# yangsenwxy/VSR

Measured on AMD Instinct MI355X. Metric: voxels/sec fwd+bwd, 4× SR on 16×128×128 cine volumes, 1/2/4/8 MI355X, higher is better.
Workload: dtype bf16

## Files before the change

### vsr_amd/build.py

```python
from __future__ import annotations

import hashlib
import os
import re
import subprocess
from concurrent.futures import ThreadPoolExecutor
from pathlib import Path

ROOT = Path(__file__).resolve().parent
CSRC = ROOT / "csrc"
LIBDIR = ROOT / "_lib"
LIB = LIBDIR / "libvsrk.so"
INCLUDE = ROOT.parent / "include"
ARCH = os.environ.get("VSRK_ARCH", "gfx950")
HIPCC = os.environ.get("HIPCC", "/opt/rocm/bin/hipcc")
FLAGS = ["-O3", "-fPIC", "-std=c++17", f"--offload-arch={ARCH}", "-Wno-unused-result"]
SRC_FLAGS = {"conv_roll.hip": ["-fno-slp-vectorize"], "conv_roll_fold.hip": ["-fno-slp-vectorize"],
             "conv_wgrad_roll.hip": ["-fno-slp-vectorize"]}


def sources() -> list[Path]:
    return sorted(CSRC.glob("*.hip"))


def _digest() -> str:
    h = hashlib.sha256()
    for p in sources() + sorted(CSRC.glob("*.h")) + sorted(INCLUDE.glob("*.h")):
        h.update(p.name.encode())
        h.update(p.read_bytes())
    h.update(" ".join(FLAGS).encode())
    h.update(repr(sorted(SRC_FLAGS.items())).encode())
    return h.hexdigest()[:16]


_INC = re.compile(r'^\s*#\s*include\s+"([^"]+)"', re.M)


def _includes(src: Path) -> list[Path]:
    seen: dict[Path, None] = {}
    todo = [src]
    while todo:
        cur = todo.pop()
        for name in _INC.findall(cur.read_text()):
            p = (cur.parent / name).resolve()
            if p.exists() and p not in seen:
                seen[p] = None
                todo.append(p)
    return sorted(seen)


def is_current() -> bool:
    stamp = LIBDIR / "libvsrk.stamp"
    return LIB.exists() and stamp.exists() and stamp.read_text() == _digest()


def build(force: bool = False, verbose: bool = False) -> Path:
    LIBDIR.mkdir(exist_ok=True)
    stamp = LIBDIR / "libvsrk.stamp"
    digest = _digest()
    if not force and LIB.exists() and stamp.exists() and stamp.read_text() == digest:
        return LIB
    objdir = LIBDIR / "obj"
    objdir.mkdir(exist_ok=True)

    def compile_one(src: Path) -> Path:
        obj = objdir / (src.stem + ".o")
        deps = b"".join(p.read_bytes() for p in _includes(src))
        flags = FLAGS + SRC_FLAGS.get(src.name, [])
        key = hashlib.sha256(src.read_bytes() + deps + " ".join(flags).encode()).hexdigest()[:16]
        ostamp = objdir / (src.stem + ".stamp")
        if not force and obj.exists() and ostamp.exists() and ostamp.read_text() == key:
            return obj
        cmd = [HIPCC, *flags, "-I", str(INCLUDE), "-c", str(src), "-o", str(obj)]
        if verbose:
            print(" ".join(cmd), flush=True)
        r = subprocess.run(cmd, capture_output=True, text=True)
        if r.returncode != 0:
            raise RuntimeError(f"hipcc failed for {src.name}:\n{r.stderr[-6000:]}")
        ostamp.write_text(key)
        return obj

    with ThreadPoolExecutor(max_workers=min(8, len(sources()))) as ex:
        objs = list(ex.map(compile_one, sources()))
    tmp = LIB.with_suffix(".so.tmp")
    cmd = [HIPCC, "-shared", f"--offload-arch={ARCH}", *[str(o) for o in objs], "-o", str(tmp)]
    r = subprocess.run(cmd, capture_output=True, text=True)
    if r.returncode != 0:
        raise RuntimeError(f"link failed:\n{r.stderr[-6000:]}")
    os.replace(tmp, LIB)
    stamp.write_text(digest)
    return LIB


if __name__ == "__main__":
    print(build(force=True, verbose=True))
```

### vsr_amd/csrc/conv_fast.hip

```cpp
#include <cstdlib>
#include <string>
#include "conv_fast_impl.h"

namespace {
using namespace vsrk_conv;

int g_fast_mode = -1;

int num_cus_fast() {
  static int n = 0;
  if (n == 0) {
    int dev = 0;
    (void)hipGetDevice(&dev);
    if (hipDeviceGetAttribute(&n, hipDeviceAttributeMultiprocessorCount, dev) != hipSuccess || n <= 0) n = 256;
  }
  return n;
}

}

int vsrk_g_grid_cap = 0;

int vsrk_conv::fast_grid(int64_t ntiles) {
  int64_t g = std::min<int64_t>(ntiles, (int64_t)num_cus_fast());
  if (vsrk_g_grid_cap > 0) g = std::min<int64_t>(g, vsrk_g_grid_cap);
  return (int)std::max<int64_t>(g, 1);
}

extern "C" int vsrk_conv_set_algo(int32_t mode) {
  VSRK_CHECK(mode >= -1 && mode <= 1, "conv_set_algo: mode must be -1, 0 or 1");
  g_fast_mode = mode;
  return VSRK_OK;
}

extern int g_pw_wide_mode;

extern "C" int vsrk_conv_set_path(const char* path, int32_t mode) {
  VSRK_CHECK(path, "conv_set_path: null path");
  const std::string p(path);
  VSRK_CHECK(mode >= -1 && mode <= (p == "wgrad_row" || p == "roll_wr" ? 2 : 1),
             "conv_set_path: mode must be -1, 0 or 1 (wgrad_row, roll_wr: 2)");
  if (p == "fast") g_fast_mode = mode;
  else if (p == "thin") vsrk_g_thin_mode = mode;
  else if (p == "wgrad_pipe") vsrk_g_wgrad_pipe_mode = mode;
  else if (p == "pw") vsrk_g_pw_mode = mode;
  else if (p == "roll") vsrk_conv_set_roll_mode(mode);
  else if (p == "wgrad_roll") vsrk_conv_set_wgrad_roll_mode(mode);
  else if (p == "wgrad_row") vsrk_conv_set_wgrad_row_mode(mode);
  else if (p == "roll_wr") vsrk_conv_set_roll_wr_mode(mode);
  else if (p == "roll_fold") vsrk_conv_set_roll_fold_mode(mode);
  else if (p == "stencil") vsrk_conv_set_stencil_mode(mode);
  else if (p == "pw_wide") g_pw_wide_mode = mode;
  else VSRK_CHECK(false, "conv_set_path: unknown path '%s' (fast, pw, roll, roll_wr, roll_fold, thin, wgrad_pipe, wgrad_roll, wgrad_row, stencil)",
                  path);
  return VSRK_OK;
}

extern "C" int vsrk_conv_set_grid_cap(int32_t max_workgroups) {
  VSRK_CHECK(max_workgroups >= 0, "conv_set_grid_cap: max_workgroups must be >= 0");
  vsrk_g_grid_cap = max_workgroups;
  return VSRK_OK;
}

int vsrk_conv_fwd_fast(const vsrk_conv_desc* d, const vsrk_tensor5* x, const void* w_packed, const float* bias,
                       const float* pro_scale, const float* pro_shift, const vsrk_tensor5* residual,
                       const vsrk_tensor5* mask, const vsrk_tensor5* y, hipStream_t s) {
  if (g_fast_mode < 0) {
    const char* e = getenv("VSRK_CONV_FAST");
    g_fast_mode = (e && e[0] == '0') ? 0 : 1;
  }
  if (g_fast_mode == 0) return 0;
  if (!vsrk_is16(x->dtype)) return 0;
  if (const int rl = vsrk_conv_fwd_roll(d, x, w_packed, bias, pro_scale, pro_shift, residual, mask, y, s)) return rl;
  if (!chunk_ok(x, 2) || x->c % 8 != 0) return 0;
  const int xr = x->shuffle > 1 ? x->shuffle : 1, yr = y->shuffle > 1 ? y->shuffle : 1;
  if (xr > 1 && (x->c / (xr * xr)) % 32 != 0) return 0;
  if (yr > 1 && ((y->c / (yr * yr)) % 32 != 0 || residual || mask)) return 0;
  if (xr > 1 && d->prologue) return 0;
  if (d->kh != d->kw || (d->kh != 1 && d->kh != 3)) return 0;
  const int ye = vsrk_esize(y->dtype);
  if (((uintptr_t)y->ptr) % (4 * ye) != 0 || y->sn % 4 || y->sd % 4 || y->sh % 4 || y->sw % 4) return 0;
  if (y->c % 4 != 0 && !(y->c < 4 && !residual && !mask && !d->accumulate)) return 0;
  for (const vsrk_tensor5* t : {residual, mask}) {
    if (t && (((uintptr_t)t->ptr) % (4 * ye) != 0 || t->sn % 4 || t->sd % 4 || t->sh % 4 || t->sw % 4 ||
              t->shuffle > 1 || t->dtype != y->dtype))
      return 0;
  }
  FastArgs a;
  static int ablate = -1;
  if (ablate < 0) {
    const char* e = getenv("VSRK_FAST_ABLATE");
    ablate = e ? atoi(e) : 0;
  }
  a.ablate = ablate;
  a.x = make_view(x);
  a.y = make_view(y);
  a.res = residual ? make_view(residual) : a.y;
  a.msk = mask ? make_view(mask) : a.y;
  a.w = w_packed;
  a.bias = bias;
  a.pro_scale = pro_scale;
  a.pro_shift = pro_shift;
  a.cin = x->c;
  a.cout = y->c;
  a.cin_pad = round_up(x->c, 32);
  a.cout_pad = round_up(y->c, 128);
  a.kd = d->kd; a.pd = d->pd; a.ph = d->ph; a.pw = d->pw;
  a.prologue = d->prologue;
  a.act = d->act;
  a.accumulate = d->accumulate;
  a.has_res = residual != nullptr;
  a.has_mask = mask != nullptr;
  a.bias_r = d->bias_perm_r;
  a.out_scale = d->out_scale;
  a.act_param = d->act_param;
  a.mask_slope = d->mask_slope;
  a.tiles_w = ceil_div(y->w, TW);
  const int NT = y->c <= 32 ? 32 : (y->c <= 64 || d->kh == 3) ? 64 : 128;
  a.ntn = ceil_div(y->c, NT);
  const bool yf = y->dtype == VSRK_F32;
  const bool h16 = x->dtype == VSRK_F16;
  const bool ys = yr > 1, xs = xr > 1;
  int rc;
  if (d->kh == 1) {
    if (xs || ys) return 0;
    rc = fast_k1(a, NT, yf, h16, s);
  } else if (NT == 32) {
    if (xs || ys) return 0;
    rc = fast_k3_n32(a, yf, h16, s);
  } else if (!xs && !ys) {
    rc = fast_k3_n64(a, yf, h16, s);
  } else if (xs && !ys) {
    rc = fast_k3_n64_xs(a, yf, h16, s);
  } else if (!xs && ys) {
    rc = fast_k3_n64_ys(a, yf, h16, s);
  } else {
    return 0;
  }
  if (rc == kFastNotEligible) return 0;
  return rc == VSRK_OK ? 1 : -rc;
}
```

### vsr_amd/csrc/conv_roll.hip

```cpp
#include <cstdlib>
#include "conv_common.h"

#ifndef ROLL_NT
#define ROLL_NT 0
#endif
typedef uint32_t roll_u32x4 __attribute__((ext_vector_type(4)));
typedef int roll_v4i __attribute__((ext_vector_type(4)));
typedef __amdgpu_buffer_rsrc_t RRsrc;
constexpr uint32_t ROLL_OOB = 0x80000000u;
__device__ __forceinline__ RRsrc roll_rsrc(const void* base) {
  const uint64_t b = (uint64_t)base;
  const uint64_t u = ((uint64_t)(uint32_t)__builtin_amdgcn_readfirstlane((int)(uint32_t)(b >> 32)) << 32) |
                     (uint32_t)__builtin_amdgcn_readfirstlane((int)(uint32_t)b);
  return __builtin_amdgcn_make_buffer_rsrc((void*)u, 0, 0x7FFFFFF0, 0x00020000);
}
__device__ __forceinline__ uint4 roll_bload16(RRsrc r, uint32_t off) {
  return __builtin_bit_cast(uint4, __builtin_amdgcn_raw_buffer_load_b128(r, (int)off, 0, 0));
}
#ifndef ROLL_SWAP
#define ROLL_SWAP 1
#endif
#ifndef ROLL_PREF2D
#define ROLL_PREF2D 1
#endif
// ... 913 lines not shown
    return true;
  };
  while (step(std::integral_constant<int, 0>{}) && step(std::integral_constant<int, 1>{}) &&
         step(std::integral_constant<int, 2>{})) {
  }
  roll_wait_vmcnt<0>();
  if (ppre) settle();
  flush(ptl, pdi, true, ppre, fscr);
#ifdef ROLL_STAMP
  if (blockIdx.x < 16 && (wave == 0 || wave == 4)) {
    unsigned* o = g_roll_stamp + (blockIdx.x * 2 + (wave >> 2)) * 128;
    o[lane] = stv0;
    o[64 + lane] = stv1;
  }
#endif
  if constexpr (EM & RE_PMASK) slope_out(sacc);
}

__global__ __launch_bounds__(256) void roll_bnred_final_kernel(const float* __restrict__ ws, int ntiles, int ntn,
                                                               int cout, const float* __restrict__ invstd,
                                                               float* __restrict__ o1, float* __restrict__ o2) {
  const int c = blockIdx.x;
  if (c >= cout) return;
  const int blk = c >> 5, cc = c & 31;
  const int nt = (ntiles - blk + ntn - 1) / ntn;
  double s1 = 0.0, s2 = 0.0;
  constexpr int U = 8;
  const int n = nt * RNW;
  for (int i0 = threadIdx.x; i0 < n; i0 += 256 * U) {
    float v1[U], v2[U];
#pragma unroll
    for (int u = 0; u < U; ++u) {
      const int i = i0 + 256 * u;
      v1[u] = v2[u] = 0.f;
      if (i < n) {
        const int t = blk + ntn * (i / RNW), w = i % RNW;
        const float* p = ws + ((int64_t)t * RNW + w) * 64;
        v1[u] = p[cc];
        v2[u] = p[32 + cc];
      }
    }
#pragma unroll
    for (int u = 0; u < U; ++u) {
      s1 += v1[u];
      s2 += v2[u];
    }
  }
  __shared__ double r1[256], r2[256];
  r1[threadIdx.x] = s1;
  r2[threadIdx.x] = s2;
  __syncthreads();
  for (int k = 128; k > 0; k >>= 1) {
    if (threadIdx.x < k) {
      r1[threadIdx.x] += r1[threadIdx.x + k];
      r2[threadIdx.x] += r2[threadIdx.x + k];
    }
    __syncthreads();
  }
  if (threadIdx.x == 0) {
    o1[c] = (float)r1[0];
    o2[c] = (float)(r2[0] * (double)invstd[c]);
  }
}


int g_roll_mode = -1;
int g_roll_wr_mode = -1;

int roll_num_cus() {
  static int n = 0;
  if (n == 0) {
    int dev = 0;
    (void)hipGetDevice(&dev);
    if (hipDeviceGetAttribute(&n, hipDeviceAttributeMultiprocessorCount, dev) != hipSuccess || n <= 0) n = 256;
  }
  return n;
}

template <int KD, int NT, int PRO, int EM, int SP, typename H, int WR = 0>
int launch_roll(const RollArgs& a, size_t lds, int grid, hipStream_t s) {
  auto kern = conv_roll_kernel<KD, NT, PRO, EM, SP, H, WR>;
  (void)hipFuncSetAttribute((const void*)kern, hipFuncAttributeMaxDynamicSharedMemorySize, (int)lds);
  kern<<<grid, RNW * 64, lds, s>>>(a);
  VSRK_LAUNCH_CHECK("conv_fwd(roll)");
  return VSRK_OK;
}


}

#ifdef ROLL_FOLD_TU
int vsrk_conv_fwd_roll_fold(const vsrk_conv_desc* d, const vsrk_tensor5* x, const void* w_packed, const float* bias,
                            const float* pro_scale, const float* pro_shift, const vsrk_tensor5* y, hipStream_t s) {
  if (d->kd != 3 || d->kh != 3 || d->kw != 3 || d->pd != 0 || x->d != 3 || y->d != 1) return 0;
  if (!vsrk_is16(x->dtype) || y->dtype != x->dtype || x->shuffle > 1 || y->shuffle > 1) return 0;
  if (d->act != VSRK_ACT_NONE && d->act != VSRK_ACT_RELU) return 0;
  if (d->accumulate || d->mask_slope || d->bias_perm_r > 1) return 0;
  if (x->c % RCH != 0 || 3 * (x->c / RCH) > RMAXSUB || !chunk_ok(x, 2)) return 0;
  if (y->c % 32 != 0 || ((uintptr_t)y->ptr) % 16 != 0 || y->sn % 8 || y->sh % 8 || y->sw % 8) return 0;
  if (d->ph < 0 || d->ph > 2 || d->pw < 0 || d->pw > 2) return 0;
  if (y->h != x->h + 2 * d->ph - 2 || y->w != x->w + 2 * d->pw - 2 || y->n != x->n) return 0;
  for (const vsrk_tensor5* t : {x, y}) {
    const int64_t span = (int64_t)(t->n - 1) * t->sn + (int64_t)(t->d - 1) * t->sd +
                         (int64_t)(t->h + RFTH + 2) * t->sh + (int64_t)(t->w + 2 * RHW) * t->sw + t->c;
    if (span >= (1ll << 31) || t->sn < 0 || t->sd < 0 || t->sh < 0 || t->sw < 0) return 0;
  }
  RollArgs a;
  a.x.ptr = (char*)x->ptr;
  a.x.d = 1; a.x.h = x->h; a.x.w = x->w;
  a.x.sn = (int)x->sn; a.x.sd = (int)x->sd; a.x.sh = (int)x->sh; a.x.sw = (int)x->sw;
  a.y.ptr = (char*)y->ptr;
  a.y.d = 1; a.y.h = y->h; a.y.w = y->w;
  a.y.sn = (int)y->sn; a.y.sd = (int)y->sd; a.y.sh = (int)y->sh; a.y.sw = (int)y->sw;
  a.res = a.y;
  a.msk = a.y;
  a.w = w_packed;
  a.bias = bias;
  a.bias_r = 1;
  a.pro_scale = pro_scale;
  a.pro_shift = pro_shift;
  a.cin = 3 * x->c;
  a.cout = y->c;
  a.cin_pad = round_up(x->c, 32);
  a.cout_pad = round_up(y->c, 128);
  a.pd = 0;
  a.ph = d->ph;
  a.pw = d->pw;
  a.prologue = d->prologue;
  a.out_scale = d->out_scale;
  const int nc = x->c / RCH;
  a.nchunk = 3 * nc;
  a.fold_nc = nc;
  a.fold_wstride = 9 * a.cout_pad * a.cin_pad;
  a.fold_tab = 3 * x->c;
  a.fold_cin = x->c;
  a.act_param = nullptr;
  a.prio = 0;
  a.mask_slope = nullptr;
  a.slope_part = nullptr;
  for (int i = 0; i < a.nchunk; ++i) {
    const int kd = i / nc;
    a.spoff[i] = (int)(kd * x->sd + (i - kd * nc) * RCH);
    a.sptap[i] = (uint16_t)kd;
  }
  const int tiles_h = ceil_div(y->h, RFTH), tiles_w = ceil_div(y->w, TW), ntn = ceil_div(y->c, 32);
  const int64_t ntiles = (int64_t)y->n * tiles_h * tiles_w * ntn;
  if (ntiles == 0) return 1;
  VSRK_CHECK(ntiles < (1ll << 31), "conv_fwd(roll fold): too many tiles");
  a.dzc = 1;
  a.ntn = make_rdiv(ntn);
  a.nzc = make_rdiv(1);
  a.tiles_w = make_rdiv(tiles_w);
  a.tiles_h = make_rdiv(tiles_h);
  a.ntiles = (int)ntiles;
  using G = RollGeo<1, 1>;
  const size_t tables = (size_t)a.cout_pad * 4 + (d->prologue ? 2 * (size_t)a.fold_tab * 4 : 0);
  const size_t lds = (size_t)RNSLOT * G::SLOT + tables;
  if (lds > 160 * 1024) return 0;
  const int grid = (int)vsrk_capped_grid(std::min<int64_t>(ntiles, roll_num_cus()));
  const bool relu = d->act == VSRK_ACT_RELU;
  int rc = vsrk_dispatch16(x->dtype, [&](auto tag) {
    using H = decltype(tag);
    if (d->prologue)
      return relu ? launch_roll<1, 1, 1, RE_RELU, SP_FOLD, H>(a, lds, grid, s) : launch_roll<1, 1, 1, 0, SP_FOLD, H>(a, lds, grid, s);
    return relu ? launch_roll<1, 1, 0, RE_RELU, SP_FOLD, H>(a, lds, grid, s) : launch_roll<1, 1, 0, 0, SP_FOLD, H>(a, lds, grid, s);
  });
  if (rc == VSRK_ERR_UNSUPPORTED) return 0;
  return rc == VSRK_OK ? 1 : -rc;
}
#else

int vsrk_g_roll_dz = 0;

extern "C" int vsrk_conv_set_roll_depth(int32_t depths) {
  VSRK_CHECK(depths >= 0, "conv_set_roll_depth: depths must be >= 0");
  vsrk_g_roll_dz = depths;
  return VSRK_OK;
}

void vsrk_conv_set_roll_wr_mode(int mode) { g_roll_wr_mode = mode; }

void vsrk_conv_set_roll_mode(int mode) { g_roll_mode = mode; }

int g_roll_fold_mode = -1;
void vsrk_conv_set_roll_fold_mode(int mode) { g_roll_fold_mode = mode; }

size_t vsrk_roll_slope_ws_bytes() { return (size_t)roll_num_cus() * RNW * sizeof(double); }

static int roll_fwd_one(const vsrk_conv_desc* d, const vsrk_tensor5* x, const void* w_packed, const float* bias,
                        const float* pro_scale, const float* pro_shift, const vsrk_tensor5* residual,
                        const vsrk_tensor5* mask, const vsrk_tensor5* y, hipStream_t s, const vsrk_slope_out* slope,
                        vsrk_roll_bnred* bnred);

int vsrk_conv_fwd_roll(const vsrk_conv_desc* d, const vsrk_tensor5* x, const void* w_packed, const float* bias,
                       const float* pro_scale, const float* pro_shift, const vsrk_tensor5* residual,
                       const vsrk_tensor5* mask, const vsrk_tensor5* y, hipStream_t s, const vsrk_slope_out* slope,
                       vsrk_roll_bnred* bnred) {
  auto span = [](const vsrk_tensor5* t, int64_t n) -> int64_t {
    const int64_t r = t->shuffle > 1 ? t->shuffle : 1;
    return (n - 1) * t->sn + (int64_t)(t->d - 1) * t->sd + (int64_t)(r * (t->h + RFTH + 2) - 1) * t->sh +
           (int64_t)(r * (t->w + 2 * RHW) - 1) * t->sw + t->c;
  };
  const vsrk_tensor5* ts[4] = {x, y, residual, mask};
  auto fits = [&](int64_t n) {
    for (const vsrk_tensor5* t : ts)
      if (t && span(t, n) >= (1ll << 31)) return false;
    return true;
  };
  if (slope || bnred || x->n <= 1 || y->n != x->n || fits(x->n))
    return roll_fwd_one(d, x, w_packed, bias, pro_scale, pro_shift, residual, mask, y, s, slope, bnred);
  for (const vsrk_tensor5* t : ts)
    if (t && (t->n != x->n || t->sn < 0)) return 0;
  int nc = x->n;
  while (nc > 1 && !fits(nc)) nc = (nc + 1) / 2;
  if (!fits(nc)) return 0;
  for (int n0 = 0; n0 < x->n; n0 += nc) {
    vsrk_tensor5 c[4];
    for (int i = 0; i < 4; ++i) {
      if (!ts[i]) continue;
      c[i] = *ts[i];
      c[i].n = std::min(nc, x->n - n0);
      c[i].ptr = (char*)ts[i]->ptr + (int64_t)n0 * ts[i]->sn * vsrk_esize(ts[i]->dtype);
    }
    const int rc = roll_fwd_one(d, &c[0], w_packed, bias, pro_scale, pro_shift, residual ? &c[2] : nullptr,
                                mask ? &c[3] : nullptr, &c[1], s, nullptr, nullptr);
    if (rc == 0 && n0 == 0) return 0;
    if (rc == 0) return -VSRK_ERR_INVALID;
    if (rc < 0) return rc;
  }
  return 1;
}

static int roll_fwd_one(const vsrk_conv_desc* d, const vsrk_tensor5* x, const void* w_packed, const float* bias,
                        const float* pro_scale, const float* pro_shift, const vsrk_tensor5* residual,
                        const vsrk_tensor5* mask, const vsrk_tensor5* y, hipStream_t s, const vsrk_slope_out* slope,
                        vsrk_roll_bnred* bnred) {
  if (g_roll_mode < 0) {
    const char* e = getenv("VSRK_CONV_ROLL");
    g_roll_mode = !e ? 2 : (e[0] == '0' ? 0 : 1);
  }
  if (g_roll_fold_mode < 0) {
    const char* e = getenv("VSRK_ROLL_FOLD");
    g_roll_fold_mode = (e && e[0] == '0') ? 0 : 1;
  }
  if (g_roll_mode == 0) return 0;
  if (!vsrk_is16(x->dtype) || y->dtype != x->dtype) return 0;
  if (d->kh != 3 || d->kw != 3) return 0;
  const bool k3 = d->kd == 3;
  if (!k3 && !(d->kd == 1 && d->pd == 0 && y->c % 64 == 0)) return 0;
  const bool pmask = slope != nullptr;
  if ((d->bias_perm_r > 1 && (y->shuffle != d->bias_perm_r || y->c % (d->bias_perm_r * d->bias_perm_r))) ||
      (d->mask_slope && !pmask))
    return 0;
  if (pmask) {
    if (!mask || !d->mask_slope || residual || d->kd != 1 || d->prologue) return 0;
    if (mask->dtype != y->dtype || mask->shuffle != y->shuffle || mask->n != y->n || mask->d != y->d ||
        mask->h != y->h || mask->w != y->w || mask->c != y->c || mask->sn != y->sn ||
        (y->d > 1 && mask->sd != y->sd) ||
        mask->sh != y->sh || mask->sw != y->sw)
      return 0;
  }
  if (d->act == VSRK_ACT_PRELU && (k3 || !d->act_param)) return 0;
  if (k3 && (residual || mask || d->accumulate)) return 0;
  if (k3 && y->d == 1 && x->d == 3 && d->pd == 0 && !bnred && !residual && !mask && !pmask && g_roll_fold_mode != 0) {
    if (const int rf = vsrk_conv_fwd_roll_fold(d, x, w_packed, bias, pro_scale, pro_shift, y, s)) return rf;
  }
  if (g_roll_mode == 2 && k3 && y->d == 1 && !bnred && vsrk_g_roll_dz == 0) return 0;
  if (bnred) {
    const vsrk_tensor5* b = bnred->bnx;
    if (!k3 || d->prologue || d->act != VSRK_ACT_NONE || bias || d->out_scale != 1.f || !b || b->dtype != y->dtype ||
        b->shuffle > 1 ||
        b->n != y->n || b->d != y->d || b->h != y->h || b->w != y->w || b->c != y->c || b->sn != y->sn ||
        b->sd != y->sd || b->sh != y->sh || b->sw != y->sw)
      return 0;
  }
  const int sp = x->shuffle > 1 ? SP_X : (y->shuffle > 1 ? SP_Y : SP_NONE);
  if (x->shuffle > 1 && y->shuffle > 1) return 0;
  if (sp != SP_NONE) {
    if (k3 || d->prologue || residual || (mask && !pmask)) return 0;
    const vsrk_tensor5* t = sp == SP_X ? x : y;
    const int r = t->shuffle, cph = t->c / (r * r);
    if (cph * r * r != t->c || cph % (sp == SP_X ? RCH : 32) != 0) return 0;
    if (t->c / (sp == SP_X ? RCH : 32) > RMAXSUB) return 0;
  }
  if (x->c % RCH != 0 || !chunk_ok(x, 2)) return 0;
  if (d->pd < 0 || d->pd > 2 || d->ph < 0 || d->ph > 2 || d->pw < 0 || d->pw > 2) return 0;
  if (y->d != x->d + 2 * d->pd - (d->kd - 1) || y->h != x->h + 2 * d->ph - 2 || y->w != x->w + 2 * d->pw - 2) return 0;
  auto out_ok = [&](const vsrk_tensor5* t) {
    return t->dtype == y->dtype && (t->shuffle <= 1 || (t == y && sp == SP_Y)) && t->n == y->n && t->d == y->d &&
           t->h == y->h && t->w == y->w &&
           t->c == y->c && ((uintptr_t)t->ptr) % 8 == 0 && t->sn % 4 == 0 && t->sd % 4 == 0 && t->sh % 4 == 0 &&
           t->sw % 4 == 0;
  };
  if (y->c % (k3 ? 8 : 4) != 0 || !out_ok(y)) return 0;
  if ((residual && !out_ok(residual)) || (mask && !pmask && !out_ok(mask))) return 0;
  for (const vsrk_tensor5* t : {x, y, residual, mask}) {
    if (!t) continue;
    const int64_t r = t->shuffle > 1 ? t->shuffle : 1;
    const int64_t span = (int64_t)(t->n - 1) * t->sn + (int64_t)(t->d - 1) * t->sd +
                         (int64_t)(r * (t->h + RFTH + 2) - 1) * t->sh + (int64_t)(r * (t->w + 2 * RHW) - 1) * t->sw +
                         t->c;
    if (span >= (1ll << 31) || t->sn < 0 || t->sd < 0 || t->sh < 0 || t->sw < 0) return 0;
  }
  auto rview = [](const vsrk_tensor5* t) {
    RView v;
    const int r = t->shuffle > 1 ? t->shuffle : 1;
    v.ptr = (char*)t->ptr;
    v.d = t->d; v.h = t->h; v.w = t->w;
    v.sn = (int)t->sn; v.sd = (int)t->sd; v.sh = (int)(r * t->sh); v.sw = (int)(r * t->sw);
    return v;
  };
  RollArgs a;
  a.x = rview(x);
  a.y = rview(y);
  a.res = rview(residual ? residual : y);
  a.msk = rview(mask ? mask : y);
  a.w = w_packed;
  a.bias = bias;
  a.bias_r = d->bias_perm_r > 1 ? d->bias_perm_r : 1;
  a.pro_scale = pro_scale;
  a.pro_shift = pro_shift;
  a.cin = x->c;
  a.cout = y->c;
  a.cin_pad = round_up(x->c, 32);
  a.cout_pad = round_up(y->c, 128);
  a.pd = d->pd;
  a.ph = d->ph;
  a.pw = d->pw;
  a.prologue = d->prologue;
  a.out_scale = d->out_scale;
  a.nchunk = x->c / RCH;
  a.act_param = d->act_param;
  {
    static int prio = -1;
    if (prio < 0) {
      const char* e = getenv("VSRK_ROLL_PRIO");
      prio = (e && e[0] == '1') ? 1 : 0;
    }
    a.prio = prio;
  }
  if (sp != SP_NONE) {
    const vsrk_tensor5* t = sp == SP_X ? x : y;
    const int r = t->shuffle, cph = t->c / (r * r), step = sp == SP_X ? RCH : 32;
    for (int i = 0; i < t->c / step; ++i) {
      const int c = i * step, sub = c / cph, cc = c - sub * cph;
      a.spoff[i] = (int)((sub / r) * t->sh + (sub % r) * t->sw + cc);
      a.sptap[i] = subpixel_tapmask(d->subpixel, r, sub);
    }
  }
  const int nt = k3 ? 1 : 2;
  const int tiles_h = ceil_div(y->h, RFTH), tiles_w = ceil_div(y->w, TW), ntn = ceil_div(y->c, 32 * nt);
  const int64_t spatial = (int64_t)y->n * tiles_h * tiles_w * ntn;
  if (spatial == 0 || y->d == 0) return 1;
  int dzc = y->d;
  if (vsrk_g_roll_dz > 0) {
    dzc = std::min(vsrk_g_roll_dz, y->d);
  } else if (k3) {
    const int64_t want = 2 * (int64_t)roll_num_cus();
    if (spatial < want) {
      const int64_t runs = std::min<int64_t>(ceil_div64(want, spatial), y->d);
      dzc = (int)ceil_div64(y->d, runs);
    }
  } else {
    dzc = 1;
  }
  a.dzc = dzc;
  const int nzc = ceil_div(y->d, dzc);
  a.ntn = make_rdiv(ntn);
  a.nzc = make_rdiv(nzc);
  a.tiles_w = make_rdiv(tiles_w);
  a.tiles_h = make_rdiv(tiles_h);
  const int64_t ntiles = spatial * nzc;
  VSRK_CHECK(ntiles < (1ll << 31), "conv_fwd(roll): too many tiles");
  a.ntiles = (int)ntiles;
  if (g_roll_wr_mode < 0) {
    const char* e = getenv("VSRK_ROLL_WRES");
    g_roll_wr_mode = (e && e[0] == '0') ? 0 : 1;
  }
  const int wres_mode = g_roll_wr_mode;
  const size_t nb = k3 ? RollGeo<3, 1>::NB : RollGeo<1, 2>::NB;
  const size_t wbytes = (size_t)a.nchunk * nb * 1024;
  const size_t tables = (size_t)a.cout_pad * 4 + (d->prologue || bnred ? 2 * (size_t)a.cin_pad * 4 : 0) +
                        (bnred ? 4 * (size_t)a.cout_pad * 4 : 0);
  const size_t wslot = k3 ? RollGeo<3, 1, 1>::SLOT : RollGeo<1, 2, 1>::SLOT;
  const bool pref2d =
      wres_mode != 2 && !k3 && ((residual != nullptr) != (mask != nullptr && !pmask)) && !d->accumulate;
  const bool wr = wres_mode && sp == SP_NONE && !d->prologue && wbytes <= 80 * 1024 && !pref2d &&
                  (k3 ? dzc == y->d : ntn == 1) && (size_t)RNSLOT * wslot + wbytes + tables <= 160 * 1024;
  const size_t slot = wr ? wslot : (k3 ? RollGeo<3, 1>::SLOT : RollGeo<1, 2>::SLOT);
  const size_t lds = (size_t)RNSLOT * slot + (wr ? wbytes : 0) + tables;
  if (bnred) {
    if (bnred->ws_floats < (size_t)ntiles * RNW * 64) return 0;
    a.bnx = (const char*)bnred->bnx->ptr;
    a.msk = rview(bnred->bnx);
    a.bn_sc = bnred->scale;
    a.bn_sh = bnred->shift;
    a.bn_mu = bnred->mean;
    a.bn_is = bnred->invstd;
    a.red_ws = bnred->ws;
    bnred->ntiles = (int)ntiles;
    bnred->ntn = ntn;
  }
  if (lds > 160 * 1024) return 0;
  const int grid = (int)vsrk_capped_grid(std::min<int64_t>(ntiles, roll_num_cus()));
  const bool relu = d->act == VSRK_ACT_RELU;
  const int em = (residual ? RE_RES : 0) | (mask ? (pmask ? RE_PMASK : RE_MASK) : 0) | (d->accumulate ? RE_ACC : 0) |
                 (relu ? RE_RELU : 0) | (d->act == VSRK_ACT_PRELU ? RE_PRELU : 0);
  a.mask_slope = d->mask_slope;
  if (pmask) {
    if ((size_t)grid * RNW > slope->cap) return 0;
    a.slope_part = slope->part;
    *slope->nparts = grid * RNW;
  }
  int rc = vsrk_dispatch16(x->dtype, [&](auto tag) {
    using H = decltype(tag);
    if (k3) {
      if (bnred)
        return wr ? launch_roll<3, 1, 0, RE_BNRED, SP_NONE, H, 1>(a, lds, grid, s)
                  : launch_roll<3, 1, 0, RE_BNRED, SP_NONE, H>(a, lds, grid, s);
      if (d->prologue) return relu ? launch_roll<3, 1, 1, RE_RELU, SP_NONE, H>(a, lds, grid, s) : launch_roll<3, 1, 1, 0, SP_NONE, H>(a, lds, grid, s);
      if (wr)
        return relu ? launch_roll<3, 1, 0, RE_RELU, SP_NONE, H, 1>(a, lds, grid, s)
                    : launch_roll<3, 1, 0, 0, SP_NONE, H, 1>(a, lds, grid, s);
      return relu ? launch_roll<3, 1, 0, RE_RELU, SP_NONE, H>(a, lds, grid, s) : launch_roll<3, 1, 0, 0, SP_NONE, H>(a, lds, grid, s);
    }
    if (d->prologue) {
      if (sp != SP_NONE || em != 0) return (int)VSRK_ERR_UNSUPPORTED;
      return launch_roll<1, 2, 1, 0, SP_NONE, H>(a, lds, grid, s);
    }
    if (sp == SP_X) {
      switch (em) {
        case 0: return launch_roll<1, 2, 0, 0, SP_X, H>(a, lds, grid, s);
        case RE_PRELU: return launch_roll<1, 2, 0, RE_PRELU, SP_X, H>(a, lds, grid, s);
        case RE_ACC: return launch_roll<1, 2, 0, RE_ACC, SP_X, H>(a, lds, grid, s);
        case RE_PMASK: return launch_roll<1, 2, 0, RE_PMASK, SP_X, H>(a, lds, grid, s);
        case RE_PMASK | RE_ACC: return launch_roll<1, 2, 0, RE_PMASK | RE_ACC, SP_X, H>(a, lds, grid, s);
        default: return (int)VSRK_ERR_UNSUPPORTED;
      }
    }
    if (sp == SP_Y) {
      switch (em) {
        case 0: return launch_roll<1, 2, 0, 0, SP_Y, H>(a, lds, grid, s);
        case RE_PRELU: return launch_roll<1, 2, 0, RE_PRELU, SP_Y, H>(a, lds, grid, s);
        case RE_ACC: return launch_roll<1, 2, 0, RE_ACC, SP_Y, H>(a, lds, grid, s);
        case RE_PMASK: return launch_roll<1, 2, 0, RE_PMASK, SP_Y, H>(a, lds, grid, s);
        case RE_PMASK | RE_ACC: return launch_roll<1, 2, 0, RE_PMASK | RE_ACC, SP_Y, H>(a, lds, grid, s);
        default: return (int)VSRK_ERR_UNSUPPORTED;
      }
    }
    if (wr) {
      switch (em) {
        case 0: return launch_roll<1, 2, 0, 0, SP_NONE, H, 1>(a, lds, grid, s);
        case RE_RELU: return launch_roll<1, 2, 0, RE_RELU, SP_NONE, H, 1>(a, lds, grid, s);
        case RE_RES | RE_ACC: return launch_roll<1, 2, 0, RE_RES | RE_ACC, SP_NONE, H, 1>(a, lds, grid, s);
        case RE_PMASK: return launch_roll<1, 2, 0, RE_PMASK, SP_NONE, H, 1>(a, lds, grid, s);
        default: return (int)VSRK_ERR_UNSUPPORTED;
      }
    }
    switch (em) {
      case 0: return launch_roll<1, 2, 0, 0, SP_NONE, H>(a, lds, grid, s);
      case RE_RELU: return launch_roll<1, 2, 0, RE_RELU, SP_NONE, H>(a, lds, grid, s);
      case RE_RES: return launch_roll<1, 2, 0, RE_RES, SP_NONE, H>(a, lds, grid, s);
      case RE_MASK: return launch_roll<1, 2, 0, RE_MASK, SP_NONE, H>(a, lds, grid, s);
      case RE_RES | RE_ACC: return launch_roll<1, 2, 0, RE_RES | RE_ACC, SP_NONE, H>(a, lds, grid, s);
      case RE_PMASK: return launch_roll<1, 2, 0, RE_PMASK, SP_NONE, H>(a, lds, grid, s);
      default: return (int)VSRK_ERR_UNSUPPORTED;
    }
  });
  if (rc == VSRK_ERR_UNSUPPORTED) return 0;
  return rc == VSRK_OK ? 1 : -rc;
}

#ifdef ROLL_STAMP
extern "C" int vsrk_roll_stamps(unsigned* dst) {
  return hipMemcpyFromSymbol(dst, HIP_SYMBOL(g_roll_stamp), sizeof(g_roll_stamp)) == hipSuccess ? 0 : 1;
}
#endif

extern "C" size_t vsrk_conv_prelu_bwd_workspace(void) {
  return std::max(vsrk_roll_slope_ws_bytes(), vsrk_pw_pbwd_ws_bytes());
}

extern "C" int vsrk_conv_fwd_prelu_bwd(const vsrk_conv_desc* d, const vsrk_tensor5* x, const void* w_packed,
                                       const float* bias, const vsrk_tensor5* y_fwd, const vsrk_tensor5* y,
                                       int32_t c_lo, float* da, int32_t accumulate_da, void* workspace,
                                       size_t workspace_bytes, void* stream) {
  VSRK_CHECK(d && x && y && y_fwd && w_packed && d->mask_slope, "conv_fwd_prelu_bwd: null argument");
  VSRK_CHECK(workspace && workspace_bytes >= vsrk_conv_prelu_bwd_workspace(),
             "conv_fwd_prelu_bwd: workspace %zu < %zu bytes", workspace_bytes, vsrk_conv_prelu_bwd_workspace());
  VSRK_CHECK(((uintptr_t)workspace & 15) == 0, "conv_fwd_prelu_bwd: workspace must be 16-byte aligned");
  VSRK_CHECK(c_lo >= 0 && c_lo < y->c, "conv_fwd_prelu_bwd: c_lo %d outside [0, %d)", c_lo, y->c);
  hipStream_t s = (hipStream_t)stream;
  if ((int64_t)y->n * y->d * y->h * y->w == 0) {
    if (da && !accumulate_da) (void)hipMemsetAsync(da, 0, sizeof(float), s);
    return VSRK_OK;
  }
  int nparts = 0;
  const vsrk_slope_out so{(double*)workspace, workspace_bytes / sizeof(double), &nparts};
  int rc;
  if (d->kd == 1 && d->kh == 1 && d->kw == 1) {
    if (bias) return VSRK_ERR_UNSUPPORTED;
    rc = vsrk_conv_fwd_pw_pbwd(d, x, w_packed, y_fwd, y, c_lo, &so, s);
  } else {
    if (c_lo != 0) return VSRK_ERR_UNSUPPORTED;
    rc = vsrk_conv_fwd_roll(d, x, w_packed, bias, nullptr, nullptr, nullptr, y_fwd, y, s, &so);
  }
  if (rc == 0) return VSRK_ERR_UNSUPPORTED;
  if (rc < 0) return -rc;
  if (da) {
    vsrk_slope_final((const double*)workspace, nparts, d->mask_slope, da, accumulate_da, 0, s);
    VSRK_LAUNCH_CHECK("conv_fwd_prelu_bwd_final");
  }
  return VSRK_OK;
}

int vsrk_roll_bnred_final(const vsrk_roll_bnred& r, int cout, float* sum_dy, float* sum_dy_xhat, hipStream_t s) {
  roll_bnred_final_kernel<<<cout, 256, 0, s>>>(r.ws, r.ntiles, r.ntn, cout, r.invstd, sum_dy, sum_dy_xhat);
  VSRK_LAUNCH_CHECK("conv_fwd_reduce(roll) final");
  return VSRK_OK;
}

size_t vsrk_roll_bnred_ws_floats(const vsrk_tensor5* y) {
  return (size_t)y->n * ceil_div(y->h, RFTH) * ceil_div(y->w, TW) * ceil_div(y->c, 32) * std::max(y->d, 1) * RNW * 64;
}
#endif
```

### vsr_amd/csrc/vsrk_internal.h

```cpp
#pragma once
#include <algorithm>
#include "vsrk_common.h"

size_t vsrk_channel_reduce_ws_bytes(int c);
int vsrk_channel_reduce_internal(const vsrk_tensor5* x, int mode, int perm_r, float scale, float* sum,
                                 float* sumsq, int accumulate, void* ws, size_t ws_bytes, hipStream_t s);

int vsrk_conv_fwd_fast(const vsrk_conv_desc* d, const vsrk_tensor5* x, const void* w_packed, const float* bias,
                       const float* pro_scale, const float* pro_shift, const vsrk_tensor5* residual,
                       const vsrk_tensor5* mask, const vsrk_tensor5* y, hipStream_t s);
int vsrk_conv_fwd_stencil(const vsrk_conv_desc* d, const vsrk_tensor5* x, const void* w_packed, const float* bias,
                          const vsrk_tensor5* residual, const vsrk_tensor5* mask, const vsrk_tensor5* y,
                          hipStream_t s);
int vsrk_conv_fwd_stencil_out(const vsrk_conv_desc* d, const vsrk_tensor5* x, const void* w_packed,
                              const float* bias, const vsrk_tensor5* residual, const vsrk_tensor5* mask,
                              const vsrk_tensor5* y, hipStream_t s);
void vsrk_conv_set_stencil_mode(int mode);
int vsrk_conv_fwd_thin(const vsrk_conv_desc* d, const vsrk_tensor5* x, const void* w_packed, const float* bias,
                       const float* pro_scale, const float* pro_shift, const vsrk_tensor5* residual,
                       const vsrk_tensor5* mask, const vsrk_tensor5* y, hipStream_t s);

struct vsrk_roll_bnred {
  const vsrk_tensor5* bnx;
  const float *scale, *shift, *mean, *invstd;
  float* ws;
  size_t ws_floats;
  int ntiles, ntn;
};
struct vsrk_slope_out {
  double* part;
  size_t cap;
  int* nparts;
};
void vsrk_slope_final(const double* part, int nparts, const float* a, float* da, int accumulate, int pre,
                      hipStream_t s);
int vsrk_conv_fwd_roll(const vsrk_conv_desc* d, const vsrk_tensor5* x, const void* w_packed, const float* bias,
                       const float* pro_scale, const float* pro_shift, const vsrk_tensor5* residual,
                       const vsrk_tensor5* mask, const vsrk_tensor5* y, hipStream_t s,
                       const vsrk_slope_out* slope = nullptr, vsrk_roll_bnred* bnred = nullptr);
int vsrk_roll_bnred_final(const vsrk_roll_bnred& r, int cout, float* sum_dy, float* sum_dy_xhat, hipStream_t s);
size_t vsrk_roll_bnred_ws_floats(const vsrk_tensor5* y);
size_t vsrk_roll_slope_ws_bytes();
void vsrk_conv_set_roll_mode(int mode);
void vsrk_conv_set_roll_wr_mode(int mode);
void vsrk_conv_set_roll_fold_mode(int mode);
int vsrk_conv_fwd_roll_fold(const vsrk_conv_desc* d, const vsrk_tensor5* x, const void* w_packed, const float* bias,
                            const float* pro_scale, const float* pro_shift, const vsrk_tensor5* y, hipStream_t s);

int vsrk_conv_fwd_pw(const vsrk_conv_desc* d, const vsrk_tensor5* x, const void* w_packed, const float* bias,
                     const float* pro_scale, const float* pro_shift, const vsrk_tensor5* residual,
                     const vsrk_tensor5* mask, const vsrk_tensor5* y, hipStream_t s);
int vsrk_conv_fwd_pw_wide(const vsrk_conv_desc* d, const vsrk_tensor5* x, const void* w_packed, const float* bias,
                          const vsrk_tensor5* residual, const vsrk_tensor5* mask, const vsrk_tensor5* y,
                          hipStream_t s);
int vsrk_conv_fwd_pw_pbwd(const vsrk_conv_desc* d, const vsrk_tensor5* x, const void* w_packed,
                          const vsrk_tensor5* mask, const vsrk_tensor5* y, int c_lo, const vsrk_slope_out* slope,
                          hipStream_t s);
size_t vsrk_pw_pbwd_ws_bytes();
size_t vsrk_conv_wgrad_pw_workspace(const vsrk_conv_desc* d, const vsrk_tensor5* x, const vsrk_tensor5* dy);
int vsrk_conv_wgrad_pw(const vsrk_conv_desc* d, const vsrk_tensor5* x, const vsrk_tensor5* dy,
                       const float* pro_scale, const float* pro_shift, float dy_scale, int32_t perm_r, float* dw,
                       float* dbias, int32_t accumulate, void* workspace, size_t workspace_bytes, hipStream_t s);

extern int vsrk_g_pw_mode;
extern int vsrk_g_thin_mode;
extern int vsrk_g_wgrad_pipe_mode;
extern int vsrk_g_grid_cap;
static inline int64_t vsrk_capped_grid(int64_t g) {
  return vsrk_g_grid_cap > 0 ? std::max<int64_t>(1, std::min<int64_t>(g, vsrk_g_grid_cap)) : g;
}
```

Measured before the change: 57.75 million.

## Add row-streaming 3x3 conv kernel for 64-channel 2D convs in roll path

```diff
diff --git a/vsr_amd/build.py b/vsr_amd/build.py
--- a/vsr_amd/build.py
+++ b/vsr_amd/build.py
@@ -16,7 +16,7 @@
 HIPCC = os.environ.get("HIPCC", "/opt/rocm/bin/hipcc")
 FLAGS = ["-O3", "-fPIC", "-std=c++17", f"--offload-arch={ARCH}", "-Wno-unused-result"]
 SRC_FLAGS = {"conv_roll.hip": ["-fno-slp-vectorize"], "conv_roll_fold.hip": ["-fno-slp-vectorize"],
-             "conv_wgrad_roll.hip": ["-fno-slp-vectorize"]}
+             "conv_wgrad_roll.hip": ["-fno-slp-vectorize"], "conv_row.hip": ["-fno-slp-vectorize"]}
 
 
 def sources() -> list[Path]:
diff --git a/vsr_amd/csrc/conv_fast.hip b/vsr_amd/csrc/conv_fast.hip
--- a/vsr_amd/csrc/conv_fast.hip
+++ b/vsr_amd/csrc/conv_fast.hip
@@ -51,7 +51,8 @@
   else if (p == "roll_fold") vsrk_conv_set_roll_fold_mode(mode);
   else if (p == "stencil") vsrk_conv_set_stencil_mode(mode);
   else if (p == "pw_wide") g_pw_wide_mode = mode;
-  else VSRK_CHECK(false, "conv_set_path: unknown path '%s' (fast, pw, roll, roll_wr, roll_fold, thin, wgrad_pipe, wgrad_roll, wgrad_row, stencil)",
+  else if (p == "row") vsrk_conv_set_row_mode(mode);
+  else VSRK_CHECK(false, "conv_set_path: unknown path '%s' (fast, pw, pw_wide, roll, roll_wr, roll_fold, row, thin, wgrad_pipe, wgrad_roll, wgrad_row, stencil)",
                   path);
   return VSRK_OK;
 }
diff --git a/vsr_amd/csrc/conv_roll.hip b/vsr_amd/csrc/conv_roll.hip
--- a/vsr_amd/csrc/conv_roll.hip
+++ b/vsr_amd/csrc/conv_roll.hip
@@ -1239,6 +1239,13 @@
                          t->c;
     if (span >= (1ll << 31) || t->sn < 0 || t->sd < 0 || t->sh < 0 || t->sw < 0) return 0;
   }
+  if (g_roll_wr_mode < 0) {
+    const char* e = getenv("VSRK_ROLL_WRES");
+    g_roll_wr_mode = (e && e[0] == '0') ? 0 : 1;
+  }
+  if (!k3 && sp == SP_NONE && !pmask && !bnred && g_roll_wr_mode == 1) {
+    if (const int rw = vsrk_conv_fwd_row(d, x, w_packed, bias, residual, mask, y, s)) return rw;
+  }
   auto rview = [](const vsrk_tensor5* t) {
     RView v;
     const int r = t->shuffle > 1 ? t->shuffle : 1;
@@ -1310,10 +1317,6 @@
   const int64_t ntiles = spatial * nzc;
   VSRK_CHECK(ntiles < (1ll << 31), "conv_fwd(roll): too many tiles");
   a.ntiles = (int)ntiles;
-  if (g_roll_wr_mode < 0) {
-    const char* e = getenv("VSRK_ROLL_WRES");
-    g_roll_wr_mode = (e && e[0] == '0') ? 0 : 1;
-  }
   const int wres_mode = g_roll_wr_mode;
   const size_t nb = k3 ? RollGeo<3, 1>::NB : RollGeo<1, 2>::NB;
   const size_t wbytes = (size_t)a.nchunk * nb * 1024;
diff --git a/vsr_amd/csrc/conv_row.hip b/vsr_amd/csrc/conv_row.hip
--- /dev/null
+++ b/vsr_amd/csrc/conv_row.hip
@@ -0,0 +1,353 @@
+#include <cstdlib>
+#include "conv_common.h"
+
+namespace {
+using namespace vsrk_conv;
+
+constexpr int CR_NW = 8;
+constexpr int CR_SEG = 128;
+constexpr int CR_SLOT = (CR_SEG + 2) * 128;
+constexpr int CR_NSLOT = 4;
+constexpr int CR_BIAS = CR_NSLOT * CR_SLOT;
+constexpr int CR_LDS = CR_BIAS + 256;
+constexpr int CR_MINBAND = 4;
+constexpr uint32_t CR_OOB = 0x80000000u;
+enum { CE_RES = 1, CE_MASK = 2, CE_ACC = 4, CE_RELU = 8 };
+
+typedef __amdgpu_buffer_rsrc_t CrRsrc;
+typedef int cr_v4i __attribute__((ext_vector_type(4)));
+__device__ __forceinline__ CrRsrc cr_rsrc(const void* base) {
+  const uint64_t b = (uint64_t)base;
+  const uint64_t u = ((uint64_t)(uint32_t)__builtin_amdgcn_readfirstlane((int)(uint32_t)(b >> 32)) << 32) |
+                     (uint32_t)__builtin_amdgcn_readfirstlane((int)(uint32_t)b);
+  return __builtin_amdgcn_make_buffer_rsrc((void*)u, 0, 0x7FFFFFF0, 0x00020000);
+}
+__device__ __forceinline__ uint4 cr_load16(CrRsrc r, uint32_t voff, uint32_t soff) {
+  return __builtin_bit_cast(uint4, __builtin_amdgcn_raw_buffer_load_b128(r, (int)voff, (int)soff, 0));
+}
+__device__ __forceinline__ void cr_store16(CrRsrc r, uint32_t voff, uint4 v) {
+  __builtin_amdgcn_raw_buffer_store_b128(__builtin_bit_cast(cr_v4i, v), r, (int)voff, 0, 0);
+}
+
+struct CrView {
+  const char* ptr;
+  int64_t sn, sd;
+  int sh, sw;
+};
+
+struct ConvRowArgs {
+  CrView x, y, res, msk;
+  const void* w;
+  const float* bias;
+  int cout_pad, cin_pad;
+  float out_scale;
+  int D, H, W;
+  int nseg, nband, band_h, nitems;
+};
+
+template <int EM, bool HALO, typename H>
+__global__ __launch_bounds__(CR_NW * 64, 1) void conv_row_kernel(ConvRowArgs a) {
+  extern __shared__ __attribute__((aligned(16))) char lds[];
+  const int tid = threadIdx.x, lane = tid & 63, r = lane & 31, hf = lane >> 5;
+  const int wave = __builtin_amdgcn_readfirstlane(tid >> 6);
+  const int coh = wave & 1, vq = wave >> 1;
+
+  uint4 wf[9][4];
+  {
+    const H* wp = reinterpret_cast<const H*>(a.w);
+#pragma unroll
+    for (int t = 0; t < 9; ++t)
+#pragma unroll
+      for (int c = 0; c < 4; ++c)
+        wf[t][c] = *reinterpret_cast<const uint4*>(wp + ((int64_t)(t * a.cout_pad + coh * 32 + r) * a.cin_pad + c * 16 + 8 * hf));
+  }
+  const int ecc = 2 * (r >> 4) + hf;
+  const int ech = coh * 32 + 8 * ecc;
+  const float osc = a.out_scale;
+  float* lbias = reinterpret_cast<float*>(lds + CR_BIAS);
+  if (tid < 64) lbias[tid] = a.bias ? a.bias[tid] * osc : 0.f;
+  if constexpr (!HALO) {
+    if (tid < CR_NSLOT * 16)
+      *reinterpret_cast<uint4*>(lds + (tid >> 4) * CR_SLOT + ((tid >> 3) & 1) * (CR_SEG + 1) * 128 + (tid & 7) * 16) =
+          make_uint4(0, 0, 0, 0);
+  }
+
+  uint32_t fa[3], fh[3];
+#pragma unroll
+  for (int kw = 0; kw < 3; ++kw) {
+    const int lv = vq * 32 + r + kw, sz = (lv >> 1) & 7;
+    fa[kw] = (uint32_t)(lv * 128 + ((hf ^ (sz & 1)) << 4));
+    fh[kw] = (uint32_t)(sz >> 1);
+  }
+  const int sp = lane & 7;
+  constexpr int NSQ = HALO ? 3 : 2;
+  const int scol = 8 * wave + (lane >> 3);
+  const int hcol = (lane >> 3) == 0 ? -1 : CR_SEG;
+  const uint32_t sdst = (uint32_t)((scol + 1) * 128 + ((sp ^ (((scol + 1) >> 1) & 7)) << 4));
+  const uint32_t hdst = (uint32_t)((hcol + 1) * 128 + ((sp ^ (((hcol + 1) >> 1) & 7)) << 4));
+  const bool halo_lane = wave == 0 && lane < 16;
+
+  f32x16 b0, b1;
+
+  for (int item = blockIdx.x; item < a.nitems; item += gridDim.x) {
+    const int band = item % a.nband;
+    const int t1 = item / a.nband;
+    const int seg = t1 % a.nseg, img = t1 / a.nseg;
+    const int in_ = img / a.D, id = img - in_ * a.D;
+    const int c0 = seg * CR_SEG;
+    const int r0 = band * a.band_h, r1 = min(r0 + a.band_h, a.H);
+    const int nstage = r1 - r0 + 1;
+
+    const CrRsrc rx = cr_rsrc(reinterpret_cast<const H*>(a.x.ptr) + (in_ * a.x.sn + id * a.x.sd));
+    const CrRsrc ry = cr_rsrc(reinterpret_cast<const H*>(a.y.ptr) + (in_ * a.y.sn + id * a.y.sd));
+    const CrRsrc rr = cr_rsrc(reinterpret_cast<const H*>(a.res.ptr) + (in_ * a.res.sn + id * a.res.sd));
+    const CrRsrc rm = cr_rsrc(reinterpret_cast<const H*>(a.msk.ptr) + (in_ * a.msk.sn + id * a.msk.sd));
+
+    const uint32_t xcolb = 2u * (uint32_t)((c0 + scol) * a.x.sw + 8 * sp);
+    const uint32_t hcolb = 2u * (uint32_t)((c0 + hcol) * a.x.sw + 8 * sp);
+    bool xok[3];
+    xok[0] = c0 + scol < a.W;
+    xok[1] = c0 + scol + 64 < a.W;
+    xok[2] = halo_lane && c0 + hcol >= 0 && c0 + hcol < a.W;
+    const int ecol = c0 + vq * 32 + (r & 15);
+    const uint32_t ycolb = 2u * (uint32_t)(ecol * a.y.sw + ech);
+    const uint32_t rcolb = 2u * (uint32_t)(ecol * a.res.sw + ech);
+    const uint32_t mcolb = 2u * (uint32_t)(ecol * a.msk.sw + ech);
+    const bool yok[2] = {ecol < a.W, ecol + 16 < a.W};
+
+    uint4 stq[CR_NSLOT][NSQ];
+    auto load_row = [&](int row, uint4 (&st)[NSQ]) __attribute__((always_inline)) {
+      const bool rv = row >= 0 && row < a.H && row <= r1;
+      const uint32_t rb = rv ? 2u * (uint32_t)(row * a.x.sh) : 0u;
+#pragma unroll
+      for (int q = 0; q < 2; ++q) st[q] = cr_load16(rx, (rv && xok[q]) ? xcolb : CR_OOB, rb + 2u * (uint32_t)(64 * q * a.x.sw));
+      if constexpr (HALO) st[2] = cr_load16(rx, (rv && xok[2]) ? hcolb : CR_OOB, rb);
+    };
+    auto write_row = [&](int slot, const uint4 (&st)[NSQ]) __attribute__((always_inline)) {
+      char* sl = lds + slot * CR_SLOT;
+#pragma unroll
+      for (int q = 0; q < 2; ++q) *reinterpret_cast<uint4*>(sl + sdst + q * 64 * 128) = st[q];
+      if constexpr (HALO) {
+        if (halo_lane) *reinterpret_cast<uint4*>(sl + hdst) = st[NSQ - 1];
+      }
+    };
+
+    uint4 pr[2], pm[2], po[2];
+    auto load_pre = [&](int orow) __attribute__((always_inline)) {
+      const bool rv = orow >= r0 && orow < r1;
+#pragma unroll
+      for (int q = 0; q < 2; ++q) {
+        const bool ok = rv && yok[q];
+        const int ro = rv ? orow : 0;
+        if constexpr (EM & CE_RES) pr[q] = cr_load16(rr, ok ? rcolb : CR_OOB, 2u * (uint32_t)(ro * a.res.sh + 16 * q * a.res.sw));
+        if constexpr (EM & CE_MASK) pm[q] = cr_load16(rm, ok ? mcolb : CR_OOB, 2u * (uint32_t)(ro * a.msk.sh + 16 * q * a.msk.sw));
+        if constexpr (EM & CE_ACC) po[q] = cr_load16(ry, ok ? ycolb : CR_OOB, 2u * (uint32_t)(ro * a.y.sh + 16 * q * a.y.sw));
+      }
+    };
+
+    auto flush = [&](const f32x16& A, int orow) __attribute__((always_inline)) {
+      const bool rv = orow >= r0 && orow < r1;
+      float v[16];
+#pragma unroll
+      for (int i = 0; i < 16; ++i) v[i] = A[i];
+#pragma unroll
+      for (int g = 0; g < 4; g += 2) {
+#pragma unroll
+        for (int i = 0; i < 4; ++i) {
+          const auto sw = __builtin_amdgcn_permlane32_swap(__builtin_bit_cast(uint32_t, v[4 * g + i]),
+                                                           __builtin_bit_cast(uint32_t, v[4 * g + 4 + i]), false, false);
+          v[4 * g + i] = __builtin_bit_cast(float, (uint32_t)sw[0]);
+          v[4 * g + 4 + i] = __builtin_bit_cast(float, (uint32_t)sw[1]);
+        }
+      }
+#pragma unroll
+      for (int e = 0; e < 8; ++e) {
+        const auto sw = __builtin_amdgcn_permlane16_swap(__builtin_bit_cast(uint32_t, v[e]),
+                                                         __builtin_bit_cast(uint32_t, v[8 + e]), false, false);
+        v[e] = __builtin_bit_cast(float, (uint32_t)sw[0]);
+        v[8 + e] = __builtin_bit_cast(float, (uint32_t)sw[1]);
+      }
+      float bsv[8];
+      {
+        const float4 c0 = *reinterpret_cast<const float4*>(lbias + ech);
+        const float4 c1 = *reinterpret_cast<const float4*>(lbias + ech + 4);
+        bsv[0] = c0.x; bsv[1] = c0.y; bsv[2] = c0.z; bsv[3] = c0.w;
+        bsv[4] = c1.x; bsv[5] = c1.y; bsv[6] = c1.z; bsv[7] = c1.w;
+      }
+#pragma unroll
+      for (int q = 0; q < 2; ++q) {
+        float t[8];
+#pragma unroll
+        for (int e = 0; e < 8; ++e) {
+          t[e] = fmaf(v[8 * q + e], osc, bsv[e]);
+          if constexpr (EM & CE_RELU) t[e] = fmaxf(t[e], 0.f);
+        }
+        if constexpr (EM & CE_MASK) {
+          float m[8];
+          Chunk<H>::unpack(pm[q], m);
+#pragma unroll
+          for (int e = 0; e < 8; ++e) t[e] = m[e] > 0.f ? t[e] : 0.f;
+        }
+        if constexpr (EM & CE_RES) {
+          float rs[8];
+          Chunk<H>::unpack(pr[q], rs);
+#pragma unroll
+          for (int e = 0; e < 8; ++e) t[e] += rs[e];
+        }
+        if constexpr (EM & CE_ACC) {
+          float o[8];
+          Chunk<H>::unpack(po[q], o);
+#pragma unroll
+          for (int e = 0; e < 8; ++e) t[e] += o[e];
+        }
+        const uint32_t yo = ycolb + 2u * (uint32_t)((rv ? orow : 0) * a.y.sh + 16 * q * a.y.sw);
+        cr_store16(ry, (rv && yok[q]) ? yo : CR_OOB, Chunk<H>::pack(t));
+      }
+    };
+
+    __syncthreads();
+    load_row(r0 - 1, stq[0]);
+    load_row(r0, stq[1]);
+    load_row(r0 + 1, stq[2]);
+    load_row(r0 + 2, stq[3]);
+    write_row(0, stq[0]);
+    write_row(1, stq[1]);
+    write_row(2, stq[2]);
+    load_pre(r0 - 1);
+
+    int s = 0;
+    auto step = [&](auto k_c, f32x16& Pcur, const f32x16& Pprev) __attribute__((always_inline)) -> bool {
+      constexpr int K = decltype(k_c)::value;
+      const int o = r0 + s;
+      __syncthreads();
+      load_row(o + 3, stq[K]);
+      flush(Pprev, o - 1);
+      load_pre(o);
+#pragma unroll
+      for (int kw = 0; kw < 3; ++kw) asm volatile("" : "+v"(fh[kw]));
+#pragma unroll
+      for (int c = 0; c < 4; ++c) {
+#pragma unroll
+        for (int kw = 0; kw < 3; ++kw) {
+          const uint32_t fo = fa[kw] + (((uint32_t)c ^ fh[kw]) << 5);
+#pragma unroll
+          for (int kh = 0; kh < 3; ++kh) {
+            const uint4 f = *reinterpret_cast<const uint4*>(lds + ((K + kh) % CR_NSLOT) * CR_SLOT + fo);
+            if (c == 0 && kw == 0 && kh == 0) {
+#pragma unroll
+              for (int k = 0; k < 16; ++k) Pcur[k] = 0.f;
+            }
+            mma<H>(Pcur, wf[kh * 3 + kw][c], f);
+          }
+        }
+      }
+      write_row((K + 3) % CR_NSLOT, stq[(K + 3) % CR_NSLOT]);
+      return ++s < nstage;
+    };
+#pragma unroll
+    for (int k = 0; k < 16; ++k) b0[k] = b1[k] = 0.f;
+    while (step(std::integral_constant<int, 0>{}, b0, b1) && step(std::integral_constant<int, 1>{}, b1, b0) &&
+           step(std::integral_constant<int, 2>{}, b0, b1) && step(std::integral_constant<int, 3>{}, b1, b0)) {
+    }
+  }
+}
+
+unsigned long long g_row_launches = 0;
+
+int cr_env_mode() {
+  const char* e = getenv("VSRK_CONV_ROW");
+  return !e ? -1 : (e[0] == '0' ? 0 : 1);
+}
+const int g_row_env = cr_env_mode();
+int g_row_mode = g_row_env;
+
+int cr_num_cus() {
+  static int n = 0;
+  if (n == 0) {
+    int dev = 0;
+    (void)hipGetDevice(&dev);
+    if (hipDeviceGetAttribute(&n, hipDeviceAttributeMultiprocessorCount, dev) != hipSuccess || n <= 0) n = 256;
+  }
+  return n;
+}
+
+template <int EM, typename H>
+int launch_row(const ConvRowArgs& a, int grid, hipStream_t s) {
+  auto kern = a.nseg > 1 ? conv_row_kernel<EM, true, H> : conv_row_kernel<EM, false, H>;
+  (void)hipFuncSetAttribute((const void*)kern, hipFuncAttributeMaxDynamicSharedMemorySize, CR_LDS);
+  kern<<<grid, CR_NW * 64, CR_LDS, s>>>(a);
+  ++g_row_launches;
+  VSRK_LAUNCH_CHECK("conv_fwd(row)");
+  return VSRK_OK;
+}
+
+constexpr bool cr_default_on(int em) {
+  return em == 0 || em == CE_RELU || em == CE_RES || em == CE_MASK || em == (CE_RES | CE_ACC);
+}
+
+}
+
+extern "C" unsigned long long vsrk_conv_row_launches(void) { return g_row_launches; }
+
+void vsrk_conv_set_row_mode(int mode) { g_row_mode = mode < 0 ? g_row_env : mode; }
+
+int vsrk_conv_fwd_row(const vsrk_conv_desc* d, const vsrk_tensor5* x, const void* w_packed, const float* bias,
+                      const vsrk_tensor5* residual, const vsrk_tensor5* mask, const vsrk_tensor5* y, hipStream_t s) {
+  if (g_row_mode == 0) return 0;
+  if (d->kd != 1 || d->kh != 3 || d->kw != 3 || d->pd != 0 || d->ph != 1 || d->pw != 1) return 0;
+  if (x->c != 64 || y->c != 64 || x->shuffle > 1 || y->shuffle > 1) return 0;
+  if (d->prologue || d->mask_slope || d->bias_perm_r > 1 || d->subpixel) return 0;
+  if (d->act != VSRK_ACT_NONE && d->act != VSRK_ACT_RELU) return 0;
+  if (x->n != y->n || x->d != y->d || x->h != y->h || x->w != y->w) return 0;
+  const int em = (residual ? CE_RES : 0) | (mask ? CE_MASK : 0) | (d->accumulate ? CE_ACC : 0) |
+                 (d->act == VSRK_ACT_RELU ? CE_RELU : 0);
+  if (em != 0 && em != CE_RELU && em != CE_RES && em != CE_MASK && em != (CE_RES | CE_ACC)) return 0;
+  if (g_row_mode < 0 && !cr_default_on(em)) return 0;
+  if (!chunk_ok(x, 2)) return 0;
+  for (const vsrk_tensor5* t : {x, y, residual, mask}) {
+    if (!t) continue;
+    const int64_t span = (int64_t)(t->h - 1) * t->sh + (int64_t)(t->w - 1) * t->sw + 64;
+    if (t->sn < 0 || t->sd < 0 || t->sh < 0 || t->sw < 0 || 2 * span >= 0x7FFFFFF0ll) return 0;
+    if (t->sh >= (1ll << 30) || t->sw >= (1ll << 30)) return 0;
+  }
+  const int64_t nimg = (int64_t)y->n * y->d;
+  if (nimg == 0 || y->h == 0 || y->w == 0) return 1;
+  auto view = [](const vsrk_tensor5* t) {
+    CrView v;
+    v.ptr = (const char*)t->ptr;
+    v.sn = t->sn; v.sd = t->sd; v.sh = (int)t->sh; v.sw = (int)t->sw;
+    return v;
+  };
+  ConvRowArgs a;
+  a.x = view(x);
+  a.y = view(y);
+  a.res = view(residual ? residual : y);
+  a.msk = view(mask ? mask : y);
+  a.w = w_packed;
+  a.bias = bias;
+  a.cin_pad = round_up(x->c, 32);
+  a.cout_pad = round_up(y->c, 128);
+  a.out_scale = d->out_scale;
+  a.D = y->d; a.H = y->h; a.W = y->w;
+  a.nseg = ceil_div(y->w, CR_SEG);
+  const int64_t target = vsrk_capped_grid(cr_num_cus());
+  const int64_t cols = nimg * a.nseg;
+  int64_t nb = std::max<int64_t>(1, std::min<int64_t>(ceil_div64(target, cols), y->h));
+  a.band_h = (int)std::max<int64_t>(ceil_div64(y->h, nb), std::min(CR_MINBAND, y->h));
+  a.nband = ceil_div(y->h, a.band_h);
+  const int64_t nitems = cols * a.nband;
+  if (nitems >= (1ll << 31)) return 0;
+  a.nitems = (int)nitems;
+  const int grid = (int)vsrk_capped_grid(std::min<int64_t>(nitems, cr_num_cus()));
+  int rc = vsrk_dispatch16(x->dtype, [&](auto tag) {
+    using H = decltype(tag);
+    switch (em) {
+      case 0: return launch_row<0, H>(a, grid, s);
+      case CE_RELU: return launch_row<CE_RELU, H>(a, grid, s);
+      case CE_RES: return launch_row<CE_RES, H>(a, grid, s);
+      case CE_MASK: return launch_row<CE_MASK, H>(a, grid, s);
+      default: return launch_row<CE_RES | CE_ACC, H>(a, grid, s);
+    }
+  });
+  return rc == VSRK_OK ? 1 : -rc;
+}
diff --git a/vsr_amd/csrc/vsrk_internal.h b/vsr_amd/csrc/vsrk_internal.h
--- a/vsr_amd/csrc/vsrk_internal.h
+++ b/vsr_amd/csrc/vsrk_internal.h
@@ -47,6 +47,10 @@
 int vsrk_conv_fwd_roll_fold(const vsrk_conv_desc* d, const vsrk_tensor5* x, const void* w_packed, const float* bias,
                             const float* pro_scale, const float* pro_shift, const vsrk_tensor5* y, hipStream_t s);
 
+int vsrk_conv_fwd_row(const vsrk_conv_desc* d, const vsrk_tensor5* x, const void* w_packed, const float* bias,
+                      const vsrk_tensor5* residual, const vsrk_tensor5* mask, const vsrk_tensor5* y, hipStream_t s);
+void vsrk_conv_set_row_mode(int mode);
+
 int vsrk_conv_fwd_pw(const vsrk_conv_desc* d, const vsrk_tensor5* x, const void* w_packed, const float* bias,
                      const float* pro_scale, const float* pro_shift, const vsrk_tensor5* residual,
                      const vsrk_tensor5* mask, const vsrk_tensor5* y, hipStream_t s);
```

New measurement: 62.30 million (median of 6 runs). +7.9%, better.
